# cptq/SignNet-BasisNet

Measured on AMD Instinct MI355X. Metric: graphs/sec SignNet+GINE forward, ZINC batch=128 k=16, higher is better.
Workload: dtype f32

## Files before the change

signnet_basisnet_amd/csrc/fused_gnn.hip:

```cpp
#include "gnn_front.hpp"

namespace sn {

#ifdef SN_PROFILE
static __device__ int g_prof_block = 0;
#undef SN_STAMP
#undef SN_ACCUM
#define SN_STAMP(i) do { if ((int)blockIdx.x == g_prof_block && threadIdx.x == 0) g_prof[i] = clock64(); } while (0)
#define SN_ACCUM(i, t0) do { if ((int)blockIdx.x == g_prof_block && threadIdx.x == 0) g_prof[i] += clock64() - (t0); } while (0)
#endif


struct GnnStruct {
  const void* x;
  int ldx;
  const void* edge_attr;
  int lde;
  const float* rho_sum;
  const int32_t* graph_ptr;
  const int32_t* rowptr;
  const int32_t* col;
  const int32_t* eperm;
  int32_t* status;
  float* y;
// ... 171 lines not shown
      epi(rt, ot, a0 + a1, cur.e[0], cur.e[1], cur.e[2]);
      __builtin_amdgcn_sched_barrier(0);
#pragma unroll
      for (int j = 0; j < SPLIT_EPI; ++j) {
        const u32x4 v = __builtin_amdgcn_raw_buffer_load_b128(rs, voff, base + (3 * NKB + j) * 1024, 0);
        cur.e[j] = f32x4{__uint_as_float(v[0]), __uint_as_float(v[1]), __uint_as_float(v[2]), __uint_as_float(v[3])};
      }
    }
  }
}

#define GNN_FRONT 0
#include "fused_gnn_graph.hpp"
#undef GNN_FRONT
#define GNN_FRONT 1
#include "fused_gnn_graph.hpp"
#undef GNN_FRONT

template <int NT, int MODE = 0, bool FRONT = false>
__global__ __launch_bounds__(GNN_WAVES * 64, 2) void k_gnn_coop(GnnStruct S, sn_gnn_params P) {
  static_assert(!FRONT || (NT == 8 && MODE == 0), "front records: the NT = 8 GINE kernel");
  if constexpr (FRONT) {
    const int n = S.graph_ptr[blockIdx.x + 1] - S.graph_ptr[blockIdx.x];
    const int4 hdr = *reinterpret_cast<const int4*>(S.front + (size_t)blockIdx.x * (size_t)S.front_stride);
    const bool have = hdr.x == 1 && hdr.y == n && hdr.z >= 0 && hdr.z <= GNN_EMAX && hdr.w >= 0 && hdr.w <= GNN_CLS &&
                      P.n_layers * hdr.w <= S.ee_rows;
    const int T = __builtin_amdgcn_readfirstlane(have ? (n + 15) >> 4 : (n > 0 && n <= GNN_ROWS ? 0 : -1));
    switch (T) {
      case 1: gnn_graph_front<1>(S, P, hdr.z, hdr.w); break;
      case 2: gnn_graph_front<2>(S, P, hdr.z, hdr.w); break;
      case 3: gnn_graph_front<3>(S, P, hdr.z, hdr.w); break;
      case 4: gnn_graph_front<4>(S, P, hdr.z, hdr.w); break;
      case 0: gnn_graph<NT, MODE, 0>(S, P); break;
      default:
        if (threadIdx.x == 0) atomicOr(&S.status[3], n > GNN_ROWS ? 1 : 8);
        if ((int)threadIdx.x < P.n_out) S.y[(int64_t)blockIdx.x * P.n_out + threadIdx.x] = __uint_as_float(0x7fc00000u);
        break;
    }
  } else if constexpr (NT == 8 && MODE == 0) {
    const int n = S.graph_ptr[blockIdx.x + 1] - S.graph_ptr[blockIdx.x];
    switch ((n + 15) >> 4) {
      case 1: gnn_graph<NT, MODE, 1>(S, P); break;
      case 2: gnn_graph<NT, MODE, 2>(S, P); break;
      case 3: gnn_graph<NT, MODE, 3>(S, P); break;
      case 4: gnn_graph<NT, MODE, 4>(S, P); break;
      default:
        if (threadIdx.x == 0) atomicOr(&S.status[3], n > GNN_ROWS ? 1 : 8);
        if ((int)threadIdx.x < P.n_out) S.y[(int64_t)blockIdx.x * P.n_out + threadIdx.x] = __uint_as_float(0x7fc00000u);
        break;
    }
  } else {
    gnn_graph<NT, MODE>(S, P);
  }
  if (S.flags_host != nullptr) {
    __syncthreads();
    if (threadIdx.x == 0) {
      __threadfence();
      if (atomicAdd(&S.status[4], 1) == (int)gridDim.x - 1) {
        __threadfence();
        for (int i = 0; i < S.n_flags; ++i)
          S.flags_host[i] = __hip_atomic_load(&S.flags_src[i], __ATOMIC_RELAXED, __HIP_MEMORY_SCOPE_AGENT);
        __threadfence_system();
        __hip_atomic_store(&S.flags_host[S.n_flags], 1, __ATOMIC_RELEASE, __HIP_MEMORY_SCOPE_SYSTEM);
        __threadfence_system();
      }
    }
  }
}

template <int NT, int MODE = 0, bool FRONT = false>
static int launch_gnn(const GnnStruct& S, const sn_gnn_params& P, int64_t B, hipStream_t st) {
  constexpr bool DGL = MODE != 0;
  constexpr int LD = 16 * NT + 4;
  const size_t base = (size_t)2 * SP_IMAGE + (size_t)((GNN_ROWS + 1) * LD) * sizeof(float) +
                      (size_t)(GNN_ROWS + 4 + GNN_EMAX * (3 + (P.n_layers > 0 ? P.edge_nf : 0)) + GNN_CLS) * sizeof(int);
  const size_t lds_cap = 160 * 1024 - 512;
  const int ee_rows = gnn_ee_rows(NT, P.n_layers > 0 ? P.edge_nf : 0);
  GnnStruct S2 = S;
  S2.ee_rows = MODE == 2 ? GNN_ROWS : ((!DGL && P.n_layers > 0) ? ee_rows : 0);
  const size_t lds = base + (size_t)(S2.ee_rows + 1) * LD * sizeof(float);
  static bool init = false;
  if (!init) {
    const size_t lds_max = lds_cap;
    if (lds_max > 64 * 1024 &&
        hipFuncSetAttribute(reinterpret_cast<const void*>(k_gnn_coop<NT, MODE, FRONT>), hipFuncAttributeMaxDynamicSharedMemorySize,
                            (int)lds_max) != hipSuccess)
      return fail(SN_ERR_LAUNCH, "sn_gnn_fused_f32: cannot raise the dynamic LDS limit to %zu", lds_max);
    init = true;
  }
  hipLaunchKernelGGL((k_gnn_coop<NT, MODE, FRONT>), dim3((unsigned)B), dim3(GNN_WAVES * 64), lds, st, S2, P);
  return SN_OK;
}

}

using namespace sn;

#ifdef SN_PROFILE
extern "C" int sn_prof_read_gnn(long long* host) { return (int)hipMemcpyFromSymbol(host, HIP_SYMBOL(g_prof), sizeof(long long) * 64); }
extern "C" int sn_prof_set_block(int b) { return (int)hipMemcpyToSymbol(HIP_SYMBOL(g_prof_block), &b, sizeof(int)); }
#endif

static int gnn_fused_impl(const sn_gnn_params* params, const void* x, int ldx, const void* edge_attr, int lde,
                          const float* rho_sum, const int32_t* graph_ptr, int64_t B, const int32_t* rowptr,
                          const int32_t* col, const int32_t* eperm, int32_t* status, float* y,
                          const int32_t* flags_src, int n_flags, int32_t* flags_host, const void* front, void* stream) {
  SN_REQUIRE(params && x && rho_sum && graph_ptr && rowptr && status && y && B >= 0, "sn_gnn_fused_f32: null pointer");
  const sn_gnn_params& P = *params;
  SN_REQUIRE(P.d > 0 && P.d <= 128, "sn_gnn_fused_f32: hidden width %d not in (0, 128]", P.d);
  SN_REQUIRE(P.n_layers >= 0 && P.n_layers <= SN_GNN_MAX_LAYERS, "sn_gnn_fused_f32: %d layers unsupported", P.n_layers);
  SN_REQUIRE(P.n_out >= 1 && P.n_out <= 16, "sn_gnn_fused_f32: n_out=%d not in [1,16]", P.n_out);
  SN_REQUIRE(P.node_nf >= 1 && P.node_nf <= (P.node_discrete ? 10 : 16) && ldx >= P.node_nf,
             "sn_gnn_fused_f32: node feature count %d unsupported", P.node_nf);
  SN_REQUIRE(P.n_layers == 0 || (edge_attr && P.edge_nf >= 1 && P.edge_nf <= (P.edge_discrete ? 10 : 16) && lde >= P.edge_nf),
             "sn_gnn_fused_f32: edge feature count %d unsupported", P.edge_nf);
  SN_REQUIRE(P.lin_a && P.lin_b && P.head_w1 && P.head_w2, "sn_gnn_fused_f32: parameters missing");
  SN_REQUIRE(P.rho_out_w == nullptr, "sn_gnn_fused_f32: rho_out_w must be NULL — fold rho.out into lin_b (see signnet_hip.h)");
  if (P.node_discrete) { for (int f = 0; f < P.node_nf; ++f) SN_REQUIRE(P.ntab[f], "sn_gnn_fused_f32: node table %d missing", f); }
  else SN_REQUIRE(P.nw && P.n_scale && P.n_shift, "sn_gnn_fused_f32: node MLP parameters missing");
  for (int l = 0; l < P.n_layers; ++l) {
    const sn_gnn_layer& L = P.layers[l];
    SN_REQUIRE(L.w1s && L.w2s && L.eps, "sn_gnn_fused_f32: layer %d parameters missing", l);
    if (P.edge_discrete) { for (int f = 0; f < P.edge_nf; ++f) SN_REQUIRE(L.etab[f], "sn_gnn_fused_f32: layer %d edge table %d missing", l, f); }
    else SN_REQUIRE(L.ew && L.e_scale && L.e_shift, "sn_gnn_fused_f32: layer %d edge MLP parameters missing", l);
  }
  if (B == 0) return SN_OK;
  SN_REQUIRE(!flags_host || (flags_src && n_flags > 0 && n_flags <= 64), "sn_gnn_fused_f32: flag report needs flags_src and 0 < n_flags <= 64");
  SN_REQUIRE(!flags_src || n_flags >= 1, "sn_gnn_fused_f32: flags_src needs n_flags >= 1");
  SN_REQUIRE((!P.node_discrete || P.node_vocab > 0) && (P.n_layers == 0 || !P.edge_discrete || P.edge_vocab > 0),
             "sn_gnn_fused_f32: node_vocab / edge_vocab (rows of the embedding tables) missing");
  GnnStruct S{x, ldx, edge_attr, lde, rho_sum, graph_ptr, rowptr, col, eperm, status, y, 0, flags_src, n_flags, flags_host,
              P.d, P.d, nullptr, 0, nullptr, 0};
  hipStream_t st = (hipStream_t)stream;
  int rc = SN_OK;
  if (front != nullptr) {
    SN_REQUIRE(P.d == FR_D && P.node_discrete == 1 && P.node_nf == 1 && P.edge_discrete == 1 && P.edge_nf == 1 && P.n_layers >= 1,
               "sn_gnn_fused_front_f32: the front record serves d = 128 with one discrete node and one discrete edge feature column");
    SN_REQUIRE((reinterpret_cast<uintptr_t>(front) & 15) == 0, "sn_gnn_fused_front_f32: the record buffer must be 16-byte aligned");
    S.front = reinterpret_cast<const unsigned char*>(front);
    S.front_stride = front_stride(front_ee_cap(P));
    rc = launch_gnn<8, 0, true>(S, P, B, st);
    if (rc != SN_OK) return rc;
    SN_CHECK_LAUNCH("sn_gnn_fused_front_f32");
    return SN_OK;
  }
  switch ((P.d + 15) / 16) {
    case 1: rc = launch_gnn<1>(S, P, B, st); break;
    case 2: rc = launch_gnn<2>(S, P, B, st); break;
    case 3: rc = launch_gnn<3>(S, P, B, st); break;
    case 4: rc = launch_gnn<4>(S, P, B, st); break;
    case 5: rc = launch_gnn<5>(S, P, B, st); break;
    case 6: rc = launch_gnn<6>(S, P, B, st); break;
    case 7: rc = launch_gnn<7>(S, P, B, st); break;
    default: rc = launch_gnn<8>(S, P, B, st); break;
  }
  if (rc != SN_OK) return rc;
  SN_CHECK_LAUNCH("sn_gnn_fused_f32");
  return SN_OK;
}

extern "C" int sn_gnn_fused_f32(const sn_gnn_params* params, const void* x, int ldx, const void* edge_attr, int lde,
                                const float* rho_sum, const int32_t* graph_ptr, int64_t B, const int32_t* rowptr,
                                const int32_t* col, const int32_t* eperm, int32_t* status, float* y,
                                const int32_t* flags_src, int n_flags, int32_t* flags_host, void* stream) {
  return gnn_fused_impl(params, x, ldx, edge_attr, lde, rho_sum, graph_ptr, B, rowptr, col, eperm, status, y, flags_src, n_flags,
                        flags_host, nullptr, stream);
}

extern "C" int sn_gnn_fused_front_f32(const sn_gnn_params* params, const void* x, int ldx, const void* edge_attr, int lde,
                                      const float* rho_sum, const int32_t* graph_ptr, int64_t B, const int32_t* rowptr,
                                      const int32_t* col, const int32_t* eperm, int32_t* status, float* y,
                                      const int32_t* flags_src, int n_flags, int32_t* flags_host, const void* front, void* stream) {
  SN_REQUIRE(front, "sn_gnn_fused_front_f32: null record buffer");
  return gnn_fused_impl(params, x, ldx, edge_attr, lde, rho_sum, graph_ptr, B, rowptr, col, eperm, status, y, flags_src, n_flags,
                        flags_host, front, stream);
}

extern "C" int sn_gin_net_fused_f32(const sn_gnn_params* params, const void* head_mid, int pool_mean, const int64_t* atom, const float* p,
                                    int ldp, int kp, const int32_t* graph_ptr, int64_t B, const int32_t* rowptr, const int32_t* col,
                                    const int32_t* eperm, int32_t* status, float* y, const int32_t* flags_src, int n_flags, void* stream) {
  SN_REQUIRE(params && head_mid && atom && p && graph_ptr && rowptr && col && eperm && status && y && B >= 0, "sn_gin_net_fused_f32: null pointer");
  const sn_gnn_params& P = *params;
  SN_REQUIRE(P.d > 0 && P.d <= 128 && (P.d & 3) == 0, "sn_gin_net_fused_f32: padded hidden width %d must be a multiple of 4 in (0, 128]", P.d);
  SN_REQUIRE(P.n_layers >= 1 && P.n_layers <= SN_GNN_MAX_LAYERS, "sn_gin_net_fused_f32: %d layers unsupported", P.n_layers);
  SN_REQUIRE(P.n_out >= 1 && P.n_out <= 16, "sn_gin_net_fused_f32: n_out=%d not in [1,16]", P.n_out);
  SN_REQUIRE(P.node_discrete == 1 && P.node_nf == 1 && P.ntab[0] && P.node_vocab > 0, "sn_gin_net_fused_f32: one atom-type table expected");
  SN_REQUIRE(P.edge_nf == 0, "sn_gin_net_fused_f32: the GIN net has no edge term (edge_nf must be 0)");
  SN_REQUIRE(P.lin_a && P.lin_b && P.head_w1 && P.head_w2 && P.rho_out_w == nullptr, "sn_gin_net_fused_f32: parameters missing");
  SN_REQUIRE(kp >= 1 && kp <= P.d && ldp >= kp, "sn_gin_net_fused_f32: positional encoding width %d unsupported", kp);
  for (int l = 0; l < P.n_layers; ++l) {
    const sn_gnn_layer& L = P.layers[l];
// ... 46 lines not shown
```

signnet_basisnet_amd/ops.py:

```python
from __future__ import annotations

import ctypes as C
import math
import struct
from dataclasses import dataclass

import torch

from . import _lib
from ._lib import (EPI_AFFINE, EPI_BIAS, EPI_LEAKY, EPI_RELU, EPI_RELU_PRE, EPI_RESIDUAL, EPI_RESIDUAL_PRE, check, lib, ptr,
                   require_cuda, stream)

__all__ = ["KernelTimer", "KERNEL_ROOFLINE", "GraphPlan", "PlanBins", "build_plan", "pack_eig", "pack_weight", "gin_aggregate", "gine_aggregate",
           "masked_linear", "masked_colstats", "masked_affine", "masked_layernorm", "set_attention",
           "slot_sum", "embedding_sum", "segment_pool", "PackedLinear",
           "EPI_BIAS", "EPI_RELU_PRE", "EPI_AFFINE", "EPI_RELU", "EPI_RESIDUAL"]


class _NoSpan:
    def __enter__(self):
        return self

    def __exit__(self, *a):
        return False
# ... 73 lines not shown
    phi_col_bin0: torch.Tensor
    phi_col_mem: torch.Tensor
    phi_col_off: torch.Tensor
    rho_bin0: torch.Tensor
    meta: torch.Tensor
    cstruct: object
    phi_bin_mem: torch.Tensor = None


@dataclass
class GraphPlan:
    N: int
    B: int
    E: int
    kmax: int
    graph_ptr: torch.Tensor
    node_graph: torch.Tensor
    nvalid: torch.Tensor
    evoff: torch.Tensor
    rowptr: torch.Tensor
    col: torch.Tensor
    eperm: torch.Tensor
    status: torch.Tensor
    bins: PlanBins | None
    flags: torch.Tensor = None
    front: torch.Tensor = None

    def check(self):
        st = self.status.tolist()
        if st[0]:
            bits = [n for b, n in ((1, "batch not sorted"), (2, "graph id out of range"),
                                   (4, "edge endpoint out of range"), (8, "edge crosses graphs")) if st[0] & b]
            raise ValueError("malformed graph batch: " + ", ".join(bits))
        if st[5] or (st[3] & 4):
            raise IndexError(EMBEDDING_INDEX_ERROR)
        return st


class _PlanBinsC(C.Structure):
    _fields_ = [("phi_bin_col", C.c_void_p), ("phi_max_bins", C.c_int64), ("phi_col_bin0", C.c_void_p),
                ("phi_col_mem", C.c_void_p), ("phi_col_off", C.c_void_p), ("rho_bin0", C.c_void_p), ("meta", C.c_void_p),
                ("node_graph", C.c_void_p), ("phi_bin_mem", C.c_void_p)]


class _PlanEarlyC(C.Structure):
    _fields_ = [("node_ids", C.c_void_p), ("n_node_ids", C.c_int64), ("node_vocab", C.c_int64),
                ("edge_ids", C.c_void_p), ("n_edge_ids", C.c_int64), ("edge_vocab", C.c_int64),
                ("max_graph_edges", C.c_int), ("reserved", C.c_int), ("host", C.c_void_p)]


class EarlyReport:
    ERR, NMAX, DEGMAX, EDGES, PHI, RHO, IDS, DONE = 0, 1, 2, 3, 4, 5, 6, 8
    _pool = []

    def __init__(self):
        if EarlyReport._pool:
            self.t, self.v = EarlyReport._pool.pop()
        else:
            self.t = torch.zeros(16, dtype=torch.int32, pin_memory=True)
            self.v = self.t.numpy()
        self.v[:] = 0
        self.cstruct = None
        self._keep = None

    def arm(self, node_ids=None, node_vocab=0, edge_ids=None, edge_vocab=0, max_graph_edges=0):
        self._keep = (node_ids, edge_ids)
        self.cstruct = _PlanEarlyC(ptr(node_ids), 0 if node_ids is None else node_ids.numel(), int(node_vocab),
                                   ptr(edge_ids), 0 if edge_ids is None else edge_ids.numel(), int(edge_vocab),
                                   int(max_graph_edges), 0, self.t.data_ptr())
        return self

    def wait(self, timeout_s=5.0):
        v = self.v
        if not (v[8] and v[9] and v[10] and v[11]):
            import time
            t_end = time.perf_counter() + timeout_s
            while not (v[8] and v[9] and v[10] and v[11]):
                if time.perf_counter() > t_end:
                    torch.cuda.synchronize()
                    if not (v[8] and v[9] and v[10] and v[11]):
                        raise RuntimeError("sn_batch_plan_ex did not report its flags")
        return v[:8].tolist()

    def wait_nmax(self):
        v = self.v
        if not v[10]:
            import time
            t_end = time.perf_counter() + 5.0
            while not v[10]:
                if time.perf_counter() > t_end:
                    torch.cuda.synchronize()
                    if not v[10]:
                        raise RuntimeError("sn_batch_plan_ex did not report the largest graph")
        return int(v[1])

    def release(self):
        self._keep = self.cstruct = None
        EarlyReport._pool.append((self.t, self.v))


def early_supported(N: int, E: int, B: int) -> bool:
    return bool(lib().sn_batch_plan_early_supported(int(N), int(E), int(B)))


def build_plan(batch: torch.Tensor, edge_index: torch.Tensor, num_graphs: int, kmax: int = 0, bins: bool = False,
               early: "EarlyReport | None" = None, columns: bool = False, counts: torch.Tensor = None, front=None) -> GraphPlan:
    require_cuda(batch, edge_index)
    if batch.dtype != torch.int64 or edge_index.dtype != torch.int64:
        raise ValueError("build_plan: batch and edge_index must be int64 (the reference's index dtype)")
    batch = batch.contiguous()
    edge_index = edge_index.contiguous()
    N, E, B = batch.numel(), edge_index.shape[1] if edge_index.numel() else 0, int(num_graphs)
    dev = batch.device
    sizes = [B + 1, N, N, N + 1, E, E, N + 8, 8]
    mb = 0
    if bins:
        mb = int(lib().sn_phi_bins_bound(B, int(kmax)))
        sizes += [8, mb if columns else 0, (B + 1) if columns else 0, (8 * B) if columns else 0, (8 * B) if columns else 0, B + 1, 16 * mb]
    if front is not None:
        if not bins or counts is not None or not early_supported(N, E, B) or B == 0:
            front = None
        else:
            sizes += [B * (int(front[3]) // 4)]
    offs = [0]
    for s in sizes:
        offs.append(offs[-1] + ((s + 3) // 4) * 4)
    arena = torch.empty(offs[-1], dtype=torch.int32, device=dev)
    parts = [arena[offs[i]:offs[i] + sizes[i]] for i in range(len(sizes))]
    graph_ptr, node_graph, nvalid, rowptr, col, eperm, scratch, status = parts[:8]
    evoff = torch.empty(B + 1, dtype=torch.int64, device=dev)
    pb = None
    if bins:
        meta, bc, cb0, mem, off, rb0, bmem = parts[8:15]
        if columns:
            cs = _PlanBinsC(bc.data_ptr(), mb, cb0.data_ptr(), mem.data_ptr(), off.data_ptr(), rb0.data_ptr(), meta.data_ptr(),
                            node_graph.data_ptr(), bmem.data_ptr())
        else:
            bc = cb0 = mem = off = None
            cs = _PlanBinsC(None, mb, None, None, None, rb0.data_ptr(), meta.data_ptr(), node_graph.data_ptr(), bmem.data_ptr())
        pb = PlanBins(bc, mb, cb0, mem, off, rb0, meta, cs, bmem)
    if counts is not None:
        with _span("sn_batch_plan_padded"):
            check(lib().sn_batch_plan_padded(ptr(batch), N, B, ptr(edge_index), E, int(kmax), ptr(graph_ptr), ptr(node_graph),
                                             ptr(nvalid), ptr(evoff), ptr(rowptr), ptr(col), ptr(eperm), ptr(status),
                                             C.byref(pb.cstruct) if pb is not None else None, ptr(scratch),
                                             C.byref(early.cstruct) if early is not None else None, ptr(counts), stream()),
                  "sn_batch_plan_padded")
    elif front is not None:
        gp, fx, fe, _ = front
        with _span("sn_batch_plan"):
            check(lib().sn_batch_plan_front(ptr(batch), N, B, ptr(edge_index), E, int(kmax), ptr(graph_ptr), ptr(node_graph),
                                            ptr(nvalid), ptr(evoff), ptr(rowptr), ptr(col), ptr(eperm), ptr(status),
                                            C.byref(pb.cstruct), ptr(scratch), C.byref(early.cstruct) if early is not None else None,
                                            C.byref(gp), ptr(fx), fx.shape[1], ptr(fe), fe.shape[1], ptr(parts[-1]), stream()),
                  "sn_batch_plan_front")
# ... 1636 lines not shown
```

signnet_basisnet_amd/pyg.py:

```python
from __future__ import annotations

import time

import torch
import torch.nn as nn

from . import _lib as _lib_mod
from . import fused, ops

import os as _os
MAX_FUSED_GRAPHS = 6144
_NO_KERNEL_FLAGS = bool(_os.environ.get("SN_NO_KERNEL_FLAGS"))
_USE_FRONT = not _os.environ.get("SN_NO_GNN_FRONT")
N_HEAD = 4
LN_EPS = 1e-6


class MaskedBN(nn.Module):
    def __init__(self, c):
        super().__init__()
        self.bn = nn.BatchNorm1d(c)

    def reset_parameters(self):
        self.bn.reset_parameters()
# ... 369 lines not shown
def _eval_cache(module):
    key = tuple((t.data_ptr(), t._version) for t in list(module.parameters()) + list(module.buffers()))
    ent = module.__dict__.get("_sn_eval_cache")
    if ent is None or ent[0] != key:
        ent = module.__dict__["_sn_eval_cache"] = (key, {})
    return ent[1]


def _drop_eval_cache(module):
    module.__dict__.pop("_sn_eval_cache", None)


def _drop_prepared(module, incompatible_keys=None):
    module._prep = None


def host_max_nodes(data):
    N, B = int(data.batch.numel()), int(data.num_graphs)
    s = getattr(data, "sizes", None)
    if s is not None and not torch.is_tensor(s):
        return (int(max(s)) if len(s) else 0) if (len(s) == B and sum(s) == N) else None
    cands = []
    sd = getattr(data, "_slice_dict", None)
    if isinstance(sd, dict):
        cands += [sd.get(key) for key in ("x", "eigen_values", "batch")]
    cands.append(getattr(data, "ptr", None))
    for t in cands:
        if torch.is_tensor(t) and not t.is_cuda and t.dim() == 1 and t.numel() == B + 1 and B >= 1 and int(t[-1]) - int(t[0]) == N:
            return int((t[1:] - t[:-1]).max())
    return None


class SignNetGNN(ops.DropoutHolder, nn.Module):

    def __init__(self, node_feat, edge_feat, n_hid, n_out, nl_signnet, nl_gnn, nl_rho=4, ignore_eigval=False,
                 gnn_type="GINEConv", *, variant="alchemy", max_k=None):
        super().__init__()
        if gnn_type != "GINEConv":
            raise ValueError("only gnn_type='GINEConv' is on the SignNet hot path (SURVEY.md §2 row 3)")
        if variant not in ("alchemy", "gine"):
            raise ValueError("variant must be 'alchemy' or 'gine'")
        self.variant, self.max_k = variant, max_k
        self.cfg = dict(node_feat=node_feat, edge_feat=edge_feat, n_hid=n_hid, n_out=n_out,
                        nl_signnet=nl_signnet, nl_gnn=nl_gnn)
        self.nl_rho = 4 if variant == "alchemy" else 1
        self.use_fused = True
        self._matmul_precision = "highest"
        self.train_stages = True
        self.strict = True
        self.overlap_front, self.overlap_inputs_ready, self._side_streams = False, True, None
        self.attn_dropout = 0.1
        self._attn_dropout_source = self.DEFAULT_ATTN_DROPOUT_SOURCE
        self._pending, self._free_hosts, self._flags_host = [], [], None
        self.sign_net = SignNet(n_hid, nl_signnet, self.nl_rho, variant, ignore_eigval)
        self.gnn = GNN(node_feat, edge_feat, n_hid, n_out, nl_gnn, variant)
        self._prep = None
        self.register_load_state_dict_post_hook(_drop_prepared)

    @property
    def attn_dropout_source(self):
        return getattr(self, "_attn_dropout_source", "generator")

    DEFAULT_ATTN_DROPOUT_SOURCE = "generator"

    @staticmethod
    def check_attn_dropout_source(name):
        if name not in ("generator", "counter"):
            raise ValueError(f"attn_dropout_source {name!r}: \"generator\" or \"counter\"")
        return name

    @attn_dropout_source.setter
    def attn_dropout_source(self, name):
        self._attn_dropout_source = self.check_attn_dropout_source(name)

    def _dropout_active(self):
        return self.attn_dropout_source == "counter" and float(self.attn_dropout or 0.0) > 0.0

    def _attn_drop(self, snap, li):
        return None if snap is None else (self.attn_dropout, snap, ops.ATTN_DROP_SITE + li)

    @property
    def matmul_precision(self):
        return getattr(self, "_matmul_precision", "highest")

    @matmul_precision.setter
    def matmul_precision(self, name):
        d = self.cfg["n_hid"]
        served = 0 < d <= 128 and d % 4 == 0
        fused.precision_code(name, (d + 15) // 16 if served else None, what=f"this model (hidden width {d})")
        self._matmul_precision = name

    @property
    def _prec(self):
        return fused.PRECISIONS[self.matmul_precision]

    def reset_parameters(self):
        self.sign_net.reset_parameters()
        self.gnn.reset_parameters()
        self._prep = None

    def train(self, mode=True):
        self._prep = None
        out = super().train(mode)
        self._drain_status()
        return out

# ... 49 lines not shown
                            bn1=_BN(ee.norms[1].bn, fold))
        if train and self.variant != "alchemy":
            ee2 = sn.eigen_encoder2
            P["eig2"] = dict(l0=_pack(ee2.layers[0]), bn0=_BN(ee2.norms[0].bn, False), l1=_pack(ee2.layers[1]),
                             bn1=_BN(ee2.norms[1].bn, False))
        P["rho"] = []
        for tl in sn.rho.transformer_layers:
            a, f = tl.slf_attn, tl.pos_ffn
            P["rho"].append(dict(q=_pack(a.w_qs), k=_pack(a.w_ks), v=_pack(a.w_vs), fc=_pack(a.fc),
                                 ln1=(a.norm.ln.weight.detach(), a.norm.ln.bias.detach()),
                                 w1=_pack(f.w_1), w2=_pack(f.w_2),
                                 ln2=(f.norm.ln.weight.detach(), f.norm.ln.bias.detach())))
        P["rho_out"] = dict(l=_pack(sn.rho.out[0]), bn=_BN(sn.rho.out[1], fold))
        if isinstance(g.input_encoder, DiscreteEncoder):
            P["in_tabs"] = [e.weight.detach() for e in g.input_encoder.embeddings]
        else:
            P["in_mlp"] = dict(l=_pack(g.input_encoder.layers[0]), bn=_BN(g.input_encoder.norms[0], fold))
        P["lin"] = _pack(g.linear)
        P["gine"] = []
        for enc, conv, norm in zip(g.edge_encoders, g.convs, g.norms):
            d = dict(eps=conv.layer.eps.detach(), l0=_pack(conv.nn.layers[0]), bn0=_BN(conv.nn.norms[0], fold),
                     l1=_pack(conv.nn.layers[1]), bn=_BN(norm, fold))
            if isinstance(enc, DiscreteEncoder):
                d["tabs"] = [e.weight.detach() for e in enc.embeddings]
            else:
                d["emlp"] = dict(l=_pack(enc.layers[0]), bn=_BN(enc.norms[0], fold))
            P["gine"].append(d)
        oe = g.output_encoder
        P["head"] = dict(l0=_pack(oe.layers[0]), bn0=_BN(oe.norms[0], fold), l1=_pack(oe.layers[1]))
        return P

    @staticmethod
    def _flags_bad(host):
        return bool(host[0] or host[3] or host[5] or host[9] or host[13] or (host[SignNetGNN._KWORD] and host[1] > host[SignNetGNN._KWORD]))

    @staticmethod
    def _flags_error(host):
        if (host[3] & 4) or host[5]:
            return IndexError(ops.EMBEDDING_INDEX_ERROR + " — the outputs of the affected graphs are NaN")
        if host[SignNetGNN._KWORD] and host[1] > host[SignNetGNN._KWORD]:
            return ValueError(f"the batch's host-side graph sizes (largest: {host[SignNetGNN._KWORD]}) disagree with its batch vector (largest graph: "
                              f"{host[1]} nodes): eigenvector slots beyond the host-side count were dropped")
        if host[0]:
            return ValueError("an earlier batch was malformed (unsorted batch vector, graph id / edge endpoint out of range or an edge "
                              "across graphs): its outputs are NaN")
        if host[3] & 8:
            return RuntimeError("an earlier batch had a graph without nodes: the fused GINE stage returns NaN for it; set model.strict = True "
                                "(re-runs such batches layer by layer) or model.use_fused = False")
        return RuntimeError("an earlier batch had a graph too large for the fused SignNet kernels (> 64 nodes or > 192 edges): "
                            "the outputs of that batch are NaN; set model.strict = True (re-runs such batches layer by layer) or "
                            "model.use_fused = False")

    def check_last(self, wait=True):
        while self._pending:
            ev, host = self._pending[0]
            if not wait and len(self._pending) <= 4 and not self._arrived(ev, host):
                break
            self._wait_status(ev, host)
            self._pending.pop(0)
            self._free_hosts.append(host)
            if self._flags_bad(host[1]):
                self._pending.clear()
                raise self._flags_error(host[1])

    _READY = 16
    _KWORD = 24

    def check_captured(self):
        plan = getattr(self, "_captured_plan", None)
        if plan is None:
            return
        flags = plan.flags.cpu().tolist() + [0] * 16
        flags[self._KWORD] = 0 if self.max_k else int(self._captured_K)
        if self._flags_bad(flags):
            raise self._flags_error(flags)

    @classmethod
    def _arrived(cls, ev, host):
        return bool(host[1][cls._READY]) if ev is None else ev.query()

    @classmethod
    def _wait_status(cls, ev, host):
        if ev is not None:
            ev.synchronize()
            return
        view = host[1]
        t_end = time.perf_counter() + 2e-3
        while not view[cls._READY]:
            if time.perf_counter() > t_end:
                torch.cuda.synchronize()
                if not view[cls._READY]:
                    raise RuntimeError("the fused GINE kernel did not report its status flags")
                break

    def _host_flags(self):
        if self._free_hosts:
            return self._free_hosts.pop()
        t = torch.zeros(32, dtype=torch.int32, pin_memory=True)
        return t, t.numpy()

    def _post_status(self, plan):
        host = self._flags_host
        self._flags_host = None
        if host is not None:
            return None, host
        host = self._host_flags()
        n = plan.flags.numel()
        host[0][:n].copy_(plan.flags, non_blocking=True)
        ev = torch.cuda.Event()
        ev.record()
        return ev, host

    def forward(self, data, return_stages=False):
        if self.training:
            if torch.is_grad_enabled() and not return_stages and any(p.requires_grad for p in self.parameters()):
                with ops.batched_bn_counters():
                    return self._forward_grad(data)
            self._prep = None
            try:
                with ops.batched_bn_counters():
                    return self._forward(data, return_stages, train=True)
            finally:
                self._prep = None
        if self.use_fused and not return_stages and int(data.num_graphs) > MAX_FUSED_GRAPHS:
            from . import dist as D
            n = -(-int(data.num_graphs) // MAX_FUSED_GRAPHS)
            return torch.cat([self.forward(D.shard_batch(data, i, n)) for i in range(n)], 0)
        capturing = torch.cuda.is_available() and torch.cuda.is_current_stream_capturing()
        if not capturing:
            self.check_last(wait=False)
        self._early = None
        try:
            with _lib_mod.stream_scope():
                y = self._forward(data, return_stages)
        except BaseException:
            stale, self._early = self._early, None
            if stale is not None:
                try:
                    stale.wait()
                    stale.release()
                except Exception:
                    pass
            raise
        early, self._early = self._early, None
        if capturing:
            self._captured_plan, self._captured_K = self._last_plan, self._last_K
            self._last_plan = None
            return y
        if early is not None:
            fl = early.wait()
            early.release()
            E_ = ops.EarlyReport
            if fl[E_.ERR]:
                raise ValueError("malformed graph batch (unsorted batch vector, graph id / edge endpoint out of range or an edge across graphs)")
            if fl[E_.IDS]:
                raise IndexError(ops.EMBEDDING_INDEX_ERROR)
            if not self.max_k and fl[E_.NMAX] > self._last_K:
                raise ValueError(f"the batch's host-side graph sizes (largest: {self._last_K}) disagree with its batch vector (largest graph: {fl[E_.NMAX]} nodes)")
            if fl[E_.EDGES] or fl[E_.PHI] or fl[E_.RHO]:
                y = self._serve_beyond_limits(data)
        elif self.use_fused and not return_stages and self._used_fused:
            ev, host = self._post_status(self._last_plan)
            host[1][self._KWORD] = 0 if self.max_k else int(self._last_K)
            if self.strict:
                self._wait_status(ev, host)
                flags = host[1].tolist()
                self._free_hosts.append(host)
                if self._flags_bad(flags):
                    if flags[0] or flags[5] or (flags[3] & 4) or (flags[self._KWORD] and flags[1] > flags[self._KWORD]):
                        raise self._flags_error(flags)
                    y = self._serve_beyond_limits(data)
            else:
                self._pending.append((ev, host))
        self._last_plan = None
        return y

    def _serve_beyond_limits(self, data):
        from . import dist as D
        B = int(data.num_graphs)
        sizes = list(data.sizes) if hasattr(data, "sizes") and len(data.sizes) == B else torch.bincount(data.batch, minlength=B).tolist()
        if data.edge_index.numel():
            ecount = torch.bincount(data.batch[data.edge_index[1]], minlength=B).tolist()
        else:
            ecount = [0] * B
        bad = [n > fused.GNN_MAX_NODES or e > fused.GNN_MAX_EDGES for n, e in zip(sizes, ecount)]
        if not any(bad) or 2 * sum(bad) > B or min(sizes) <= 0:
            return self._forward(data, False, force_layer=True)
        runs, lo = [], 0
        for g in range(1, B + 1):
            if g == B or bad[g] != bad[lo]:
                runs.append((lo, g, bad[lo]))
                lo = g
        outs = []
        saved_strict, self.strict = self.strict, False
        try:
            for lo, hi, is_bad in runs:
                sub = D.slice_graphs(data, lo, hi, sizes)
                outs.append(self._forward(sub, False, force_layer=is_bad))
                if not is_bad and self._used_fused:
                    ev, host = self._post_status(self._last_plan)
                    host[1][self._KWORD] = 0 if self.max_k else int(self._last_K)
                    self._pending.append((ev, host))
        finally:
            self.strict = saved_strict
        return torch.cat(outs, 0)

    def _forward_grad(self, data):
        from . import autograd as AG
        ops.require_cuda(data.edge_index, data.batch, data.eigen_vectors)
        sn, g = self.sign_net, self.gnn
        B = int(data.num_graphs)
        pad = getattr(self, "_bucket", None)
        plan = ops.build_plan(data.batch, data.edge_index, B, self.max_k or (0 if pad is None else int(pad.K)),
                              counts=None if pad is None else pad.counts)
        rplan = ops.build_plan(data.batch, data.edge_index.flip(0).contiguous(), B, self.max_k or 0)
        if pad is None:
            K = int(self.max_k) if self.max_k else plan.check()[1]
            vN = vE = vB = None
            k1 = 0
        else:
            K = int(pad.K)
            vN, vE, vB, k1 = pad.node_valid, pad.edge_valid, pad.graph_valid, 1
        N, nv = plan.N, plan.nvalid
        alchemy_eig = self.variant == "alchemy" and not sn.ignore_eigval
        want_vals = alchemy_eig or self.variant != "alchemy"
        x0, s0 = ops.pack_eig(plan, data.eigen_vectors, data.eigen_values if want_vals else None, K, want_vals)

        def lin_bn(x, lin, norm, nvalid=None, K_=0, relu=True, residual=None):
            if isinstance(norm, _Identity):
                y = AG.linear(x, lin.weight, lin.bias, nvalid, K_, relu=relu)
                return y if residual is None else AG.masked_add(y, residual, nvalid, K_)
            bn = norm.bn if isinstance(norm, MaskedBN) else norm
            if stage and isinstance(bn, nn.BatchNorm1d) and T.supported(lin.weight.shape[1], lin.weight.shape[0]):
                return T.lin_bn(x, lin, bn, nvalid, K_, relu=relu, residual=residual)
            return AG.linear_bn_act(x, lin.weight, lin.bias, bn, nvalid, K_, relu=relu, residual=residual)

        from . import train_stage as T
        d = self.cfg["n_hid"]
        stage = self.train_stages and T.supported(d, d)

        def scalar_form(l0, l1):
            return stage and l0.weight.numel() == 1 and l0.bias is None and l1.weight.shape[1] == 1

        if self.variant != "alchemy":
            with torch.no_grad():
                ee2 = sn.eigen_encoder2
                if scalar_form(ee2.layers[0], ee2.layers[1]):
                    T.scalar_mlp_stats(s0, ee2.layers[0], ee2.norms[0].bn, ee2.layers[1], ee2.norms[1].bn, nv, K)
                else:
                    p2 = lin_bn(s0.view(N * K, 1), ee2.layers[0], ee2.norms[0], nv, K)
                    lin_bn(p2, ee2.layers[1], ee2.norms[1], nv, K)
        convs, norms = list(sn.phi.convs), list(sn.phi.norms)
        if stage and len(convs) > 1:
            if scalar_form(convs[0].nn.layers[0], convs[0].nn.layers[1]):
                a0 = AG.gin_aggregate(x0.view(N, -1), convs[0].layer.eps, plan, rplan)
                x = T.scalar_mlp(a0.view(-1), convs[0].nn.layers[0], convs[0].nn.norms[0].bn, convs[0].nn.layers[1], norms[0].bn, nv, K,
                                 G=2, negate_second=True)
# ... 40 lines not shown
            o = lin(o, a.fc)
            y = AG.masked_layernorm(o, x, a.norm.ln.weight, a.norm.ln.bias, LN_EPS, nv, K)
            z = lin(y, f.w_1, relu=True)
            z = lin(z, f.w_2)
            x = AG.masked_layernorm(z, y, f.norm.ln.weight, f.norm.ln.bias, LN_EPS, nv, K)
        s = AG.slot_sum(x, N, K, nv)
        pe = lin_bn(s, sn.rho.out[0], sn.rho.out[1], vN, k1, relu=False)
        xin = data.x.squeeze() if data.x.dim() > 1 and data.x.shape[-1] == 1 else data.x
        if isinstance(g.input_encoder, DiscreteEncoder):
            h = AG.embedding_sum(xin, [e.weight for e in g.input_encoder.embeddings], plan.status[5:6])
        else:
            h = lin_bn(xin.contiguous(), g.input_encoder.layers[0], g.input_encoder.norms[0], vN, k1)
        h = AG.linear(torch.cat([h, pe], dim=-1), g.linear.weight, g.linear.bias, vN, k1)
        staged = [stage and isinstance(conv.nn.norms[0], nn.BatchNorm1d) and isinstance(norm, nn.BatchNorm1d)
                  for conv, norm in zip(g.convs, g.norms)]
        e_all = None
        if all(staged) and all(isinstance(enc, DiscreteEncoder) for enc in g.edge_encoders) and 1 < len(g.edge_encoders) <= 16:
            e_all = AG.embedding_sum_layers(data.edge_attr, [[t.weight for t in enc.embeddings] for enc in g.edge_encoders], plan.status[5:6])
        for li, (enc, conv, norm) in enumerate(zip(g.edge_encoders, g.convs, g.norms)):
            if e_all is not None:
                h = T.gine_layer(h, e_all, conv.layer.eps, conv.nn.layers[0], conv.nn.norms[0], conv.nn.layers[1], norm, plan, rplan, layer=li,
                                 nvalid=vN, K=k1)
                continue
            if isinstance(enc, DiscreteEncoder):
                e = AG.embedding_sum(data.edge_attr, [t.weight for t in enc.embeddings], plan.status[5:6])
            else:
                e = lin_bn(data.edge_attr.contiguous(), enc.layers[0], enc.norms[0], vE, k1)
            if staged[li]:
                h = T.gine_layer(h, e, conv.layer.eps, conv.nn.layers[0], conv.nn.norms[0], conv.nn.layers[1], norm, plan, rplan,
                                 nvalid=vN, K=k1)
            else:
                u = AG.gine_aggregate(h, e, conv.layer.eps, plan, rplan)
                u = lin_bn(u, conv.nn.layers[0], conv.nn.norms[0], vN, k1)
                h = lin_bn(u, conv.nn.layers[1], norm, vN, k1, residual=h)
        pooled = AG.segment_pool(h, plan, g.pooling)
        oe = g.output_encoder
        y = lin_bn(pooled, oe.layers[0], oe.norms[0], vB, k1)
        y = AG.linear(y, oe.layers[1].weight, oe.layers[1].bias, vB, k1)
        discrete = isinstance(g.input_encoder, DiscreteEncoder) or any(isinstance(e, DiscreteEncoder) for e in g.edge_encoders)
        self._train_status = plan.status if discrete else None
        if not getattr(self, "_defer_status", False):
            self.check_train()
        return y

    def check_train(self):
        st, self._train_status = getattr(self, "_train_status", None), None
        if st is not None and int(st[5]):
            raise IndexError(ops.EMBEDDING_INDEX_ERROR)

    @staticmethod
    def _arm_early(gplan, data):
        xi = ei = None
        nv = ev = 0
        if gplan.node_discrete and data.x.dtype == torch.int64 and data.x.is_cuda:
            xi, nv = data.x.contiguous(), int(gplan.params.node_vocab)
        if gplan.edge_discrete and int(gplan.params.n_layers) > 0 and data.edge_attr.dtype == torch.int64 and data.edge_attr.is_cuda \
                and data.edge_attr.numel() > 0:
            ei, ev = data.edge_attr.contiguous(), int(gplan.params.edge_vocab)
        return ops.EarlyReport().arm(xi, nv, ei, ev, fused.GNN_MAX_EDGES)

    def _forward_overlapped(self, data, P, B):
        d = self.cfg["n_hid"]
        dev = data.batch.device
        cur = torch.cuda.current_stream(dev)
        if self._side_streams is None:
            self._side_streams = (torch.cuda.Stream(device=dev), torch.cuda.Stream(device=dev))
        side_a, side_b = self._side_streams
        if not self.overlap_inputs_ready:
            side_a.wait_stream(cur)
        want_vals = "eig" in P or "eig2" in P
        with torch.cuda.stream(side_a), _lib_mod.stream_scope():
            plan = ops.build_plan(data.batch, data.edge_index, B, self.max_k or 0, bins=True)
            K_host = None if self.max_k else host_max_nodes(data)
            K = int(self.max_k) if self.max_k else (int(K_host) if K_host is not None else plan.check()[1])
            x = P["phi_fused"].run(plan, data.eigen_vectors, K, zero_invalid=False, precision=self._prec).view(plan.N * K, d)
            ev_a = torch.cuda.Event()
            ev_a.record(side_a)
        side_b.wait_event(ev_a)
        with torch.cuda.stream(side_b), _lib_mod.stream_scope():
            s = P["rho_fused"].run(plan, x, data.eigen_values if want_vals else None, K, precision=self._prec, waves=4)
            ev_b = torch.cuda.Event()
            ev_b.record(side_b)
        cur.wait_event(ev_b)
        for t in (data.batch, data.edge_index, data.eigen_vectors):
            t.record_stream(side_a)
        if want_vals:
            data.eigen_values.record_stream(side_b)
        for t in (plan.graph_ptr, plan.evoff):
            t.record_stream(side_b)
            t.record_stream(cur)
        x.record_stream(side_b)
        s.record_stream(cur)
        self._last_plan, self._used_fused, self._last_K = plan, True, K
        with _lib_mod.stream_scope():
            self._flags_host = self._host_flags() if (plan.bins is not None and not _NO_KERNEL_FLAGS) else None
            if self._flags_host is not None:
                self._flags_host[1][:] = 0
            return P["gnn_fused"].run(plan, data.x, data.edge_attr, s, None if self._flags_host is None else self._flags_host[0])

    def _forward(self, data, return_stages=False, train=False, force_layer=False):
        ops.require_cuda(data.edge_index, data.batch, data.eigen_vectors)
        if self._prep is None:
            self._prep = self._prepare(train)
        P = self._prep
        B = int(data.num_graphs)
        use_phi_fused = P["phi_fused"] is not None and not force_layer
        use_rho_fused = P["rho_fused"] is not None and not force_layer
        use_gnn_fused = P["gnn_fused"] is not None and not force_layer
        if (self.overlap_front and use_phi_fused and use_rho_fused and use_gnn_fused and not return_stages and not train
                and not self.strict):
            return self._forward_overlapped(data, P, B)
        all_fused = use_phi_fused and use_rho_fused and use_gnn_fused and not return_stages and not train
        early = None
        N_, E_n = int(data.batch.numel()), (int(data.edge_index.shape[1]) if data.edge_index.numel() else 0)
        capturing = torch.cuda.is_current_stream_capturing()
        if all_fused and self.strict and not capturing and ops.early_supported(N_, E_n, B):
            early = self._arm_early(P["gnn_fused"], data)
        K_host = None if self.max_k else host_max_nodes(data)
        if not self.max_k and K_host is None and early is None and not return_stages and not capturing and ops.early_supported(N_, E_n, B):
            early = ops.EarlyReport().arm()
        front = P["gnn_fused"].front_args(data.x, data.edge_attr) if (all_fused and _USE_FRONT) else None
        plan = ops.build_plan(data.batch, data.edge_index, B, self.max_k or 0, bins=use_phi_fused or use_rho_fused, early=early,
                              front=front)
        self._last_plan, self._used_fused = plan, (use_phi_fused or use_rho_fused or use_gnn_fused)
        if self.max_k:
            K = int(self.max_k)
            plan.check() if return_stages else None
        elif K_host is not None:
            K = int(K_host)
            plan.check() if return_stages else None
        elif early is not None:
            K = early.wait_nmax()
        else:
            K = plan.check()[1]
        if early is not None and not (all_fused and self.strict):
            early.wait()
            early.release()
            early = None
        self._early, self._last_K = early, K
        N, d = plan.N, self.cfg["n_hid"]
        nv = plan.nvalid
        want_vals = "eig" in P or "eig2" in P
        x0 = s0 = None
        if return_stages or not (use_phi_fused and use_rho_fused):
            x0, s0 = ops.pack_eig(plan, data.eigen_vectors, data.eigen_values if want_vals else None, K, want_vals)
        stages = {}

        if "eig2" in P:
            E2 = P["eig2"]
            p2 = _lin_bn(s0.view(N * K, 1), E2["l0"], E2["bn0"], True, nv, K, relu=True)
            _lin_bn(p2, E2["l1"], E2["bn1"], True, nv, K, relu=True)
        phis = None
        if use_phi_fused and not return_stages:
            x = P["phi_fused"].run(plan, data.eigen_vectors, K, zero_invalid=not use_rho_fused, precision=self._prec).view(N * K, d)
        else:
            phis = []
            for sign in (0, 1):
                x, prev = x0, None
                for l, L in enumerate(P["phi"]):
                    a = ops.gin_aggregate(x.view(N, -1), plan, L["eps"], negate=(sign == 1 and l == 0))
                    h = _lin_bn(a.view(N * K, -1), L["l0"], L["bn0"], train, nv, K, relu=True)
                    x = _lin_bn(h, L["l1"], L["bn"], train, nv, K, relu=True, residual=prev)
                    prev = x
                phis.append(x)
            x = ops.masked_affine(phis[0], nv, K, residual=phis[1])
        if return_stages:
            stages.update(phi_plus=phis[0].view(N, K, d), phi_minus=phis[1].view(N, K, d), phi=x.view(N, K, d))
            if P["phi_fused"] is not None:
                stages["phi_fused"] = P["phi_fused"].run(plan, data.eigen_vectors, K, precision=self._prec)
                stages["bins_meta"] = plan.bins.meta
        x_phi = x
        if use_rho_fused and not return_stages:
            s = P["rho_fused"].run(plan, x_phi, data.eigen_values if want_vals else None, K, precision=self._prec)
        else:
            if "eig" in P:
                E_ = P["eig"]
                p = _lin_bn(s0.view(N * K, 1), E_["l0"], E_["bn0"], train, nv, K, relu=True)
                p = _lin_bn(p, E_["l1"], E_["bn1"], train, nv, K, relu=True)
                x = ops.masked_affine(x, nv, K, residual=p)
            given = getattr(self, "_attn_masks", None) if train else None
            snap = self._dropout_begin(x.device) if train and self._dropout_active() else None
            for li, L in enumerate(P["rho"]):
                q = ops.masked_linear(x, L["q"], nv, K)
                k = ops.masked_linear(x, L["k"], nv, K)
                v = ops.masked_linear(x, L["v"], nv, K)
                pm = None
                if train:
                    pm = given[li] if given is not None else None if snap is not None else \
                        ops.attention_dropout_mask(N, K, N_HEAD, self.attn_dropout, x.device)
                o = ops.set_attention(q, k, v, N, K, N_HEAD, nv, pm, None if pm is not None else self._attn_drop(snap, li))
                o = ops.masked_linear(o, L["fc"], nv, K)
                y = ops.masked_layernorm(o, x, L["ln1"][0], L["ln1"][1], LN_EPS, nv, K)
                z = ops.masked_linear(y, L["w1"], nv, K, relu=True)
                z = ops.masked_linear(z, L["w2"], nv, K)
                x = ops.masked_layernorm(z, y, L["ln2"][0], L["ln2"][1], LN_EPS, nv, K)
            s = ops.slot_sum(x, N, K)
        if use_gnn_fused and not return_stages:
            self._flags_host = self._host_flags() if (plan.bins is not None and not _NO_KERNEL_FLAGS and self._early is None) else None
            if self._flags_host is not None:
                self._flags_host[1][:] = 0
            return P["gnn_fused"].run(plan, data.x, data.edge_attr, s, None if self._flags_host is None else self._flags_host[0])
        pe = _lin_bn(s, P["rho_out"]["l"], P["rho_out"]["bn"], train, relu=False)
        if return_stages:
            stages["pos"] = pe
            stages["rho_sum"] = s
            if use_rho_fused:
                rho_in = stages["phi_fused"].view(N * K, d) if (self._prec and "phi_fused" in stages) else x_phi
                stages["rho_sum_fused"] = P["rho_fused"].run(plan, rho_in, data.eigen_values if want_vals else None, K, precision=self._prec)
        xin = data.x.squeeze() if data.x.dim() > 1 and data.x.shape[-1] == 1 else data.x
        if "in_tabs" in P:
            h = ops.embedding_sum(xin, P["in_tabs"], plan.status[5:6])
        else:
            h = _lin_bn(xin.contiguous(), P["in_mlp"]["l"], P["in_mlp"]["bn"], train, relu=True)
        h = ops.masked_linear(torch.cat([h, pe], dim=-1), P["lin"])
        for l, L in enumerate(P["gine"]):
            if "tabs" in L:
                e = ops.embedding_sum(data.edge_attr, L["tabs"], plan.status[5:6])
            else:
                e = _lin_bn(data.edge_attr.contiguous(), L["emlp"]["l"], L["emlp"]["bn"], train, relu=True)
            u = ops.gine_aggregate(h, e, plan, L["eps"])
            u = _lin_bn(u, L["l0"], L["bn0"], train, relu=True)
            h = _lin_bn(u, L["l1"], L["bn"], train, relu=True, residual=h)
            if return_stages:
                stages[f"gine{l}"] = h
        pooled = ops.segment_pool(h, plan, self.gnn.pooling)
        y = _lin_bn(pooled, P["head"]["l0"], P["head"]["bn0"], train, relu=True)
        y = ops.masked_linear(y, P["head"]["l1"])
        if ("in_tabs" in P or any("tabs" in d for d in P["gine"])) and int(plan.status[5]):
            raise IndexError(ops.EMBEDDING_INDEX_ERROR)
        if return_stages:
            stages["y"] = y
            if use_gnn_fused:
                stages["y_gnn_fused"] = P["gnn_fused"].run(plan, data.x, data.edge_attr, s)
            return y, stages
        return y
```

Measured before the change: 582,200.

## Defer early-report status checks in non-strict mode and trim host-side per-call overhead

In non-strict fused inference, the early validation report is now queued and polled on a later call instead of being waited on synchronously. This removes a host/device sync from each forward. Host work is also trimmed: the ctypes struct is reused, early_supported results are memoized, and static plan facts and the stream-capture flag are cached. The final-block flag copy in the kernel now uses a wave of threads instead of a serial loop, and the front path falls back to the generic kernel when host flags are requested. In exchange, error reporting is deferred to a later call and a limbo list of reports is added, which adds complexity and risks late or missed error delivery.

```diff
diff --git a/signnet_basisnet_amd/csrc/fused_gnn.hip b/signnet_basisnet_amd/csrc/fused_gnn.hip
--- a/signnet_basisnet_amd/csrc/fused_gnn.hip
+++ b/signnet_basisnet_amd/csrc/fused_gnn.hip
@@ -247,17 +247,23 @@
   } else {
     gnn_graph<NT, MODE>(S, P);
   }
-  if (S.flags_host != nullptr) {
-    __syncthreads();
-    if (threadIdx.x == 0) {
-      __threadfence();
-      if (atomicAdd(&S.status[4], 1) == (int)gridDim.x - 1) {
-        __threadfence();
-        for (int i = 0; i < S.n_flags; ++i)
-          S.flags_host[i] = __hip_atomic_load(&S.flags_src[i], __ATOMIC_RELAXED, __HIP_MEMORY_SCOPE_AGENT);
-        __threadfence_system();
-        __hip_atomic_store(&S.flags_host[S.n_flags], 1, __ATOMIC_RELEASE, __HIP_MEMORY_SCOPE_SYSTEM);
-        __threadfence_system();
+  if constexpr (!FRONT) {
+    if (S.flags_host != nullptr) {
+      __syncthreads();
+      if (threadIdx.x < 64) {
+        int last = 0;
+        if (threadIdx.x == 0) {
+          __threadfence();
+          last = atomicAdd(&S.status[4], 1) == (int)gridDim.x - 1;
+        }
+        if (__shfl(last, 0, 64)) {
+          __threadfence();
+          if ((int)threadIdx.x < S.n_flags)
+            S.flags_host[threadIdx.x] = __hip_atomic_load(&S.flags_src[threadIdx.x], __ATOMIC_RELAXED, __HIP_MEMORY_SCOPE_AGENT);
+          __threadfence_system();
+          if (threadIdx.x == 0)
+            __hip_atomic_store(&S.flags_host[S.n_flags], 1, __ATOMIC_RELEASE, __HIP_MEMORY_SCOPE_SYSTEM);
+        }
       }
     }
   }
@@ -332,6 +338,8 @@
     SN_REQUIRE(P.d == FR_D && P.node_discrete == 1 && P.node_nf == 1 && P.edge_discrete == 1 && P.edge_nf == 1 && P.n_layers >= 1,
                "sn_gnn_fused_front_f32: the front record serves d = 128 with one discrete node and one discrete edge feature column");
     SN_REQUIRE((reinterpret_cast<uintptr_t>(front) & 15) == 0, "sn_gnn_fused_front_f32: the record buffer must be 16-byte aligned");
+  }
+  if (front != nullptr && flags_host == nullptr) {
     S.front = reinterpret_cast<const unsigned char*>(front);
     S.front_stride = front_stride(front_ee_cap(P));
     rc = launch_gnn<8, 0, true>(S, P, B, st);
diff --git a/signnet_basisnet_amd/ops.py b/signnet_basisnet_amd/ops.py
--- a/signnet_basisnet_amd/ops.py
+++ b/signnet_basisnet_amd/ops.py
@@ -149,25 +149,55 @@
 class EarlyReport:
     ERR, NMAX, DEGMAX, EDGES, PHI, RHO, IDS, DONE = 0, 1, 2, 3, 4, 5, 6, 8
     _pool = []
+    _made = 0
 
     def __init__(self):
         if EarlyReport._pool:
-            self.t, self.v = EarlyReport._pool.pop()
+            self.t, self.v, self._cbuf = EarlyReport._pool.pop()
         else:
             self.t = torch.zeros(16, dtype=torch.int32, pin_memory=True)
             self.v = self.t.numpy()
+            self._cbuf = _PlanEarlyC(None, 0, 0, None, 0, 0, 0, 0, self.t.data_ptr())
+            EarlyReport._made += 1
         self.v[:] = 0
         self.cstruct = None
         self._keep = None
+        self.kword = 0
+
+    def poll(self):
+        w = self.v.tolist()
+        return w if (w[8] and w[9] and w[10] and w[11]) else None
+
+    def done(self):
+        return self.poll() is not None
+
+    @classmethod
+    def words_bad(cls, fl, kword=0):
+        return bool(fl[0] or fl[3] or fl[4] or fl[5] or fl[6] or (kword and fl[1] > kword))
+
+    def status_words(self, fl=None):
+        if fl is None:
+            fl = self.v.tolist()
+        w = [0] * 32
+        w[0], w[1], w[2] = fl[self.ERR], fl[self.NMAX], fl[self.DEGMAX]
+        w[3] = (1 if (fl[self.EDGES] or (fl[self.PHI] & 1)) else 0) | (4 if fl[self.IDS] else 0) | (fl[self.PHI] & 8)
+        w[9], w[13] = fl[self.PHI] & 5, fl[self.RHO]
+        w[24] = int(self.kword)
+        return w
 
     def arm(self, node_ids=None, node_vocab=0, edge_ids=None, edge_vocab=0, max_graph_edges=0):
         self._keep = (node_ids, edge_ids)
-        self.cstruct = _PlanEarlyC(ptr(node_ids), 0 if node_ids is None else node_ids.numel(), int(node_vocab),
-                                   ptr(edge_ids), 0 if edge_ids is None else edge_ids.numel(), int(edge_vocab),
-                                   int(max_graph_edges), 0, self.t.data_ptr())
+        c = self._cbuf
+        c.node_ids, c.n_node_ids, c.node_vocab = ptr(node_ids), 0 if node_ids is None else node_ids.numel(), int(node_vocab)
+        c.edge_ids, c.n_edge_ids, c.edge_vocab = ptr(edge_ids), 0 if edge_ids is None else edge_ids.numel(), int(edge_vocab)
+        c.max_graph_edges = int(max_graph_edges)
+        self.cstruct = c
         return self
 
     def wait(self, timeout_s=5.0):
+        w = self.poll()
+        if w is not None:
+            return w[:8]
         v = self.v
         if not (v[8] and v[9] and v[10] and v[11]):
             import time
@@ -193,11 +223,20 @@
 
     def release(self):
         self._keep = self.cstruct = None
-        EarlyReport._pool.append((self.t, self.v))
+        EarlyReport._pool.append((self.t, self.v, self._cbuf))
+
+
+_early_ok = {}
 
 
 def early_supported(N: int, E: int, B: int) -> bool:
-    return bool(lib().sn_batch_plan_early_supported(int(N), int(E), int(B)))
+    key = (N, E, B)
+    r = _early_ok.get(key)
+    if r is None:
+        if len(_early_ok) >= 4096:
+            _early_ok.clear()
+        r = _early_ok[key] = bool(lib().sn_batch_plan_early_supported(int(N), int(E), int(B)))
+    return r
 
 
 def build_plan(batch: torch.Tensor, edge_index: torch.Tensor, num_graphs: int, kmax: int = 0, bins: bool = False,
diff --git a/signnet_basisnet_amd/pyg.py b/signnet_basisnet_amd/pyg.py
--- a/signnet_basisnet_amd/pyg.py
+++ b/signnet_basisnet_amd/pyg.py
@@ -445,6 +445,7 @@
         self.attn_dropout = 0.1
         self._attn_dropout_source = self.DEFAULT_ATTN_DROPOUT_SOURCE
         self._pending, self._free_hosts, self._flags_host = [], [], None
+        self._limbo = []
         self.sign_net = SignNet(n_hid, nl_signnet, self.nl_rho, variant, ignore_eigval)
         self.gnn = GNN(node_feat, edge_feat, n_hid, n_out, nl_gnn, variant)
         self._prep = None
@@ -600,16 +601,42 @@
                             "model.use_fused = False")
 
     def check_last(self, wait=True):
+        if getattr(self, "_limbo", None):
+            self._sweep_limbo()
         while self._pending:
             ev, host = self._pending[0]
-            if not wait and len(self._pending) <= 4 and not self._arrived(ev, host):
-                break
-            self._wait_status(ev, host)
-            self._pending.pop(0)
-            self._free_hosts.append(host)
-            if self._flags_bad(host[1]):
+            if isinstance(host, ops.EarlyReport):
+                fl = host.poll()
+                if fl is None:
+                    if not wait and len(self._pending) <= 4:
+                        break
+                    self._wait_status(ev, host)
+                    fl = host.poll()
+                self._pending.pop(0)
+                flags = host.status_words(fl) if host.words_bad(fl, host.kword) else None
+                host.release()
+            else:
+                if not wait and len(self._pending) <= 4 and not self._arrived(ev, host):
+                    break
+                self._wait_status(ev, host)
+                self._pending.pop(0)
+                self._free_hosts.append(host)
+                flags = host[1] if self._flags_bad(host[1]) else None
+            if flags is not None and self._flags_bad(flags):
+                self._limbo = getattr(self, "_limbo", []) + [h for _, h in self._pending if isinstance(h, ops.EarlyReport)]
                 self._pending.clear()
-                raise self._flags_error(host[1])
+                self._sweep_limbo()
+                raise self._flags_error(flags)
+
+    def _sweep_limbo(self):
+        limbo = getattr(self, "_limbo", None)
+        if limbo:
+            self._limbo = []
+            for h in limbo:
+                if h.done():
+                    h.release()
+                else:
+                    self._limbo.append(h)
 
     _READY = 16
     _KWORD = 24
@@ -625,10 +652,15 @@
 
     @classmethod
     def _arrived(cls, ev, host):
+        if isinstance(host, ops.EarlyReport):
+            return host.done()
         return bool(host[1][cls._READY]) if ev is None else ev.query()
 
     @classmethod
     def _wait_status(cls, ev, host):
+        if isinstance(host, ops.EarlyReport):
+            host.wait()
+            return
         if ev is not None:
             ev.synchronize()
             return
@@ -678,24 +710,24 @@
         if not capturing:
             self.check_last(wait=False)
         self._early = None
+        self._cap = capturing
         try:
             with _lib_mod.stream_scope():
                 y = self._forward(data, return_stages)
         except BaseException:
-            stale, self._early = self._early, None
-            if stale is not None:
-                try:
-                    stale.wait()
-                    stale.release()
-                except Exception:
-                    pass
+            self._drop_early()
             raise
+        finally:
+            self._cap = None
         early, self._early = self._early, None
         if capturing:
             self._captured_plan, self._captured_K = self._last_plan, self._last_K
             self._last_plan = None
             return y
-        if early is not None:
+        if early is not None and not self.strict:
+            self._early = early
+            self._queue_status()
+        elif early is not None:
             fl = early.wait()
             early.release()
             E_ = ops.EarlyReport
@@ -723,6 +755,25 @@
         self._last_plan = None
         return y
 
+    def _drop_early(self):
+        stale, self._early = self._early, None
+        if stale is not None:
+            try:
+                stale.wait()
+                stale.release()
+            except Exception:
+                pass
+
+    def _queue_status(self):
+        early, self._early = self._early, None
+        if early is not None:
+            early.kword = 0 if self.max_k else int(self._last_K)
+            self._pending.append((None, early))
+            return
+        ev, host = self._post_status(self._last_plan)
+        host[1][self._KWORD] = 0 if self.max_k else int(self._last_K)
+        self._pending.append((ev, host))
+
     def _serve_beyond_limits(self, data):
         from . import dist as D
         B = int(data.num_graphs)
@@ -746,11 +797,10 @@
                 sub = D.slice_graphs(data, lo, hi, sizes)
                 outs.append(self._forward(sub, False, force_layer=is_bad))
                 if not is_bad and self._used_fused:
-                    ev, host = self._post_status(self._last_plan)
-                    host[1][self._KWORD] = 0 if self.max_k else int(self._last_K)
-                    self._pending.append((ev, host))
+                    self._queue_status()
         finally:
             self.strict = saved_strict
+            self._drop_early()
         return torch.cat(outs, 0)
 
     def _forward_grad(self, data):
@@ -897,11 +947,14 @@
     def _arm_early(gplan, data):
         xi = ei = None
         nv = ev = 0
-        if gplan.node_discrete and data.x.dtype == torch.int64 and data.x.is_cuda:
-            xi, nv = data.x.contiguous(), int(gplan.params.node_vocab)
-        if gplan.edge_discrete and int(gplan.params.n_layers) > 0 and data.edge_attr.dtype == torch.int64 and data.edge_attr.is_cuda \
-                and data.edge_attr.numel() > 0:
-            ei, ev = data.edge_attr.contiguous(), int(gplan.params.edge_vocab)
+        st = getattr(gplan, "_early_static", None)
+        if st is None:
+            st = gplan._early_static = (bool(gplan.node_discrete), int(gplan.params.node_vocab),
+                                        bool(gplan.edge_discrete) and int(gplan.params.n_layers) > 0, int(gplan.params.edge_vocab))
+        if st[0] and data.x.dtype == torch.int64 and data.x.is_cuda:
+            xi, nv = data.x.contiguous(), st[1]
+        if st[2] and data.edge_attr.dtype == torch.int64 and data.edge_attr.is_cuda and data.edge_attr.numel() > 0:
+            ei, ev = data.edge_attr.contiguous(), st[3]
         return ops.EarlyReport().arm(xi, nv, ei, ev, fused.GNN_MAX_EDGES)
 
     def _forward_overlapped(self, data, P, B):
@@ -958,8 +1011,10 @@
         all_fused = use_phi_fused and use_rho_fused and use_gnn_fused and not return_stages and not train
         early = None
         N_, E_n = int(data.batch.numel()), (int(data.edge_index.shape[1]) if data.edge_index.numel() else 0)
-        capturing = torch.cuda.is_current_stream_capturing()
-        if all_fused and self.strict and not capturing and ops.early_supported(N_, E_n, B):
+        capturing = getattr(self, "_cap", None)
+        if capturing is None:
+            capturing = torch.cuda.is_current_stream_capturing()
+        if all_fused and not capturing and ops.early_supported(N_, E_n, B):
             early = self._arm_early(P["gnn_fused"], data)
         K_host = None if self.max_k else host_max_nodes(data)
         if not self.max_k and K_host is None and early is None and not return_stages and not capturing and ops.early_supported(N_, E_n, B):
@@ -978,7 +1033,7 @@
             K = early.wait_nmax()
         else:
             K = plan.check()[1]
-        if early is not None and not (all_fused and self.strict):
+        if early is not None and not all_fused:
             early.wait()
             early.release()
             early = None
@@ -1041,7 +1096,8 @@
                 x = ops.masked_layernorm(z, y, L["ln2"][0], L["ln2"][1], LN_EPS, nv, K)
             s = ops.slot_sum(x, N, K)
         if use_gnn_fused and not return_stages:
-            self._flags_host = self._host_flags() if (plan.bins is not None and not _NO_KERNEL_FLAGS and self._early is None) else None
+            self._flags_host = self._host_flags() if (plan.bins is not None and not _NO_KERNEL_FLAGS and self._early is None
+                                                      and not capturing) else None
             if self._flags_host is not None:
                 self._flags_host[1][:] = 0
             return P["gnn_fused"].run(plan, data.x, data.edge_attr, s, None if self._flags_host is None else self._flags_host[0])
```

Measured after the change: 595,900, median of 6. 1.02x the previous value.
